# theopaid/Parallel-Image-Convolution-using-MPI-OPENMP-and-CUDA

Hardware: AMD Instinct MI355X
Metric: Mpixels/sec (and wall-time) for 1920x2520 RGB, 40 reps at 1/2/4/8 MI355X (higher is better)
Workload: dtype fp32-exact (packed 16-bit integer, bit-identical to the reference float32)

## Files before the change

### parallel-image-convolution-using-mpi-openmp-and-cuda_amd/csrc/kernels/stencil_swar.hip

```cpp
#include <hip/hip_runtime.h>

#include <algorithm>
#include <cmath>
#include <cstdio>
#include <cstdlib>
#include <atomic>
#include <map>
#include <mutex>
#include <string>
#include <tuple>
#include <type_traits>
#include <vector>

#include "pconv/device.hpp"
#include "swar.hpp"
#include "swar_device.hpp"
#include "tuning.hpp"

namespace pconv {
namespace {

template <int CH, int NP, int M, int NW, int FORM, bool REP>
__device__ __forceinline__ void run_steps(u32 (&D)[M][NP], uint4 (&lds)[2][NW][2][NP / 4][64], int steps, int w,
                                          int lane, bool needs_mask, const u32 (&cm)[NP], int out_top, int out_bot,
                                          const EdgeFix<CH, NP, REP>& ef) {
  if constexpr (REP)
    if (out_top > 0 || out_bot < M) edge_rows<NP, M>(D, out_top, out_bot);
  if constexpr (FORM == 1) {
    int s = 0;
    for (; s + 2 <= steps; s += 2) {
      swar_step<CH, NP, M, NW, 1, REP>(D, lds, 0, w, lane, needs_mask, cm, out_top, out_bot, ef);
      swar_step<CH, NP, M, NW, 2, REP>(D, lds, 1, w, lane, needs_mask, cm, out_top, out_bot, ef);
    }
    if (s < steps) swar_step<CH, NP, M, NW, 0, REP>(D, lds, 0, w, lane, needs_mask, cm, out_top, out_bot, ef);
  } else {
    for (int s = 0; s < steps; ++s)
      swar_step<CH, NP, M, NW, 0, REP>(D, lds, s & 1, w, lane, needs_mask, cm, out_top, out_bot, ef);
  }
}

template <int CH, int NP, int M>
__device__ __forceinline__ void edge_fix(EdgeFix<CH, NP, true>& ef, int baseA, int baseB, bool hasB, int lane,
                                         int row_bytes, int row_base, int g_row0, int height) {
  constexpr int LW = NP;
  edge_masks<CH, NP>(ef, baseA + lane * LW, baseB + lane * LW, hasB, row_bytes);
  const auto holds_edge = [&](int base) {
    return base <= 0 || (base < row_bytes && base + 64 * LW > row_bytes - CH);
  };
  ef.h = holds_edge(baseA) || (hasB && holds_edge(baseB));
  ef.above_own = -g_row0 - row_base == 0;
  ef.below_own = height - 1 - g_row0 - row_base == M - 1;
}
template <int CH, int NP, int M>
__device__ __forceinline__ void edge_fix(EdgeFix<CH, NP, false>&, int, int, bool, int, int, int, int, int) {}

template <int CH, int LW, int M, int NW, int FORM, bool REP = false>
__global__ __launch_bounds__(64 * NW) void k_swar(const uint8_t* __restrict__ src, uint8_t* __restrict__ dst,
                                                  int64_t pitch, int row_bytes, int r0, int r1,
                                                  int steps, int g_row0, int height, int nstrips, int pair_stride,
                                                  int row_tiles, int xcd_swizzle, int tiles_per_image,
                                                  int64_t batch_stride) {
  constexpr int NP = LW;
  constexpr int NQ = NP / 4;
  using CT = typename Chunk<NP>::T;
  __shared__ uint4 lds[2][NW][2][NQ][64];
  const int lane = threadIdx.x & 63;
  const int w = __builtin_amdgcn_readfirstlane(threadIdx.x >> 6);
  const int hl = (steps * CH + LW - 1) / LW;
  const int vbytes = (64 - 2 * hl) * LW;
  int tile = static_cast<int>(blockIdx.x);
  if (xcd_swizzle) {
    const int nwg = static_cast<int>(gridDim.x);
    const int q = nwg >> 3, rem = nwg & 7, xcd = tile & 7, local = tile >> 3;
    tile = xcd * q + min(xcd, rem) + local;
  }
  {
    const int img = tile / tiles_per_image;
    tile -= img * tiles_per_image;
    src += static_cast<int64_t>(img) * batch_stride;
    dst += static_cast<int64_t>(img) * batch_stride;
  }
  const int col = tile / row_tiles, rtile = tile - col * row_tiles;
  const int sA = col, sB = col + pair_stride;
  const bool hasB = sB < nstrips;
  const int baseA = sA * vbytes - hl * LW, baseB = sB * vbytes - hl * LW;
  const int xA = baseA + lane * LW, xB = baseB + lane * LW;
  const int validA = (xA >= 0) ? min(max(row_bytes - xA, 0), LW) : 0;
  const int validB = (hasB && xB >= 0) ? min(max(row_bytes - xB, 0), LW) : 0;
  const bool needs_mask = baseA < 0 || baseA + 64 * LW > row_bytes || !hasB || baseB + 64 * LW > row_bytes;
  u32 cm[NP];
#pragma unroll
  for (int k = 0; k < NP; ++k) cm[k] = (k < validA ? 0xffffu : 0u) | (k < validB ? 0xffff0000u : 0u);

  const int vrows = NW * M - 2 * steps;
  const int tile_r0 = r0 + rtile * vrows;
  const int row_base = tile_r0 - steps + w * M;
  const int lo_ok = max(r0 - steps, -g_row0), hi_ok = min(r1 + steps, height - g_row0);

  u32 D[M][NP];
#pragma unroll
  for (int i = 0; i < M; ++i) {
    const int fr = row_base + i;
    const bool rok = fr >= lo_ok && fr < hi_ok;
    CT a = Chunk<NP>::zero(), b = Chunk<NP>::zero();
    const uint8_t* rowp = src + static_cast<int64_t>(fr) * pitch;
    if (rok && validA > 0) a = *reinterpret_cast<const CT*>(rowp + xA);
    if (rok && validB > 0) b = *reinterpret_cast<const CT*>(rowp + xB);
    unpack<NP>(a, b, D[i]);
  }
  const int out_top = min(max(-g_row0 - row_base, 0), M);
  const int out_bot = min(max(height - g_row0 - row_base, 0), M);

  EdgeFix<CH, NP, REP> ef;
  edge_fix<CH, NP, M>(ef, baseA, baseB, hasB, lane, row_bytes, row_base, g_row0, height);

  run_steps<CH, NP, M, NW, FORM, REP>(D, lds, steps, w, lane, needs_mask, cm, out_top, out_bot, ef);

  const bool lane_in = lane >= hl && lane < 64 - hl;
  const bool stA = lane_in && validA > 0, stB = lane_in && validB > 0;
  const int st_lo = max(tile_r0, r0), st_hi = min(min(tile_r0 + vrows, r1), height - g_row0);
#pragma unroll
  for (int i = 0; i < M; ++i) {
    const int fr = row_base + i;
    if (fr >= st_lo && fr < st_hi) {
      CT a, b;
      pack<NP>(D[i], a, b);
      uint8_t* rowq = dst + static_cast<int64_t>(fr) * pitch;
      if (stA) {
        if (validA == LW)
          *reinterpret_cast<CT*>(rowq + xA) = a;
        else
          store_bytes<NP>(rowq + xA, a, validA);
      }
      if (stB) {
        if (validB == LW)
          *reinterpret_cast<CT*>(rowq + xB) = b;
        else
          store_bytes<NP>(rowq + xB, b, validB);
      }
    }
  }
}

template <int CH, int M, int NW, int FORM, bool REP = false>
__global__ __launch_bounds__(64 * NW) void k_swar_pf(const uint8_t* __restrict__ src, uint8_t* __restrict__ dst,
                                                     int pitch, int row_bytes, int r0, int r1,
                                                     int steps, int g_row0, int height, int nstrips, int pair_stride,
                                                     int row_tiles, int xcd_swizzle, int tiles_per_image,
                                                     int64_t batch_stride) {
  constexpr int LW = 4, NP = 4, NQ = 1;
  constexpr u32 kOut = 0x80000000u;
  __shared__ uint4 lds[2][NW][2][NQ][64];
  const int lane = threadIdx.x & 63;
  const int w = __builtin_amdgcn_readfirstlane(threadIdx.x >> 6);
  const int hl = (steps * CH + LW - 1) / LW;
  const int vbytes = (64 - 2 * hl) * LW;
  const int vrows = NW * M - 2 * steps;
  const int lo_ok = max(r0 - steps, -g_row0), hi_ok = min(r1 + steps, height - g_row0);
  const int st_end = min(r1, height - g_row0);
  int tile = static_cast<int>(blockIdx.x);
  if (xcd_swizzle) {
    const int nwg = static_cast<int>(gridDim.x);
    const int q = nwg >> 3, rem = nwg & 7, xcd = tile & 7, local = tile >> 3;
    tile = xcd * q + min(xcd, rem) + local;
  }
  {
    const int img = tile / tiles_per_image;
    tile -= img * tiles_per_image;
    src += static_cast<int64_t>(img) * batch_stride;
    dst += static_cast<int64_t>(img) * batch_stride;
  }
  const auto srsrc = __builtin_amdgcn_make_buffer_rsrc(
      const_cast<uint8_t*>(src) + static_cast<int64_t>(lo_ok) * pitch, 0, max(hi_ok - lo_ok, 0) * pitch, 0x00020000);
  const auto drsrc = __builtin_amdgcn_make_buffer_rsrc(dst + static_cast<int64_t>(r0) * pitch, 0,
                                                       max(st_end - r0, 0) * pitch, 0x00020000);
  const int col = tile / row_tiles, rtile = tile - col * row_tiles;
  const int sB = col + pair_stride;
  const int baseA = col * vbytes - hl * LW, baseB = sB * vbytes - hl * LW;
  const int pa0 = baseA + lane * LW, pb0 = baseB + lane * LW;
  const int xA = (pa0 >= 0 && pa0 < row_bytes) ? pa0 : -1;
  const int xB = (sB < nstrips && pb0 >= 0 && pb0 < row_bytes) ? pb0 : -1;
  const bool needs_mask = baseA < 0 || baseA + 64 * LW > row_bytes || sB >= nstrips || baseB + 64 * LW > row_bytes;
  const int row_base = r0 + rtile * vrows - steps + w * M;
  u32 D[M][NP];
#pragma unroll
  for (int i = 0; i < M; ++i) {
    const int fr = row_base + i;
    const bool rok = fr >= lo_ok && fr < hi_ok;
    const u32 ro = static_cast<u32>(fr - lo_ok) * static_cast<u32>(pitch);
    const u32 a = __builtin_amdgcn_raw_buffer_load_b32(srsrc, (rok && xA >= 0) ? ro + xA : kOut, 0, 0);
    const u32 b = __builtin_amdgcn_raw_buffer_load_b32(srsrc, (rok && xB >= 0) ? ro + xB : kOut, 0, 0);
    unpack<NP>(a, b, D[i]);
  }
  u32 cm[NP];
#pragma unroll
  for (int k = 0; k < NP; ++k)
    cm[k] = (xA >= 0 && xA + k < row_bytes ? 0xffffu : 0u) | (xB >= 0 && xB + k < row_bytes ? 0xffff0000u : 0u);
  const int out_top = min(max(-g_row0 - row_base, 0), M);
  const int out_bot = min(max(height - g_row0 - row_base, 0), M);
  EdgeFix<CH, NP, REP> ef;
  edge_fix<CH, NP, M>(ef, baseA, baseB, sB < nstrips, lane, row_bytes, row_base, g_row0, height);
  run_steps<CH, NP, M, NW, FORM, REP>(D, lds, steps, w, lane, needs_mask, cm, out_top, out_bot, ef);
  const bool lane_in = lane >= hl && lane < 64 - hl;
  const int tile_r0 = row_base + steps - w * M;
  const int st_lo = max(tile_r0, r0), st_hi = min(tile_r0 + vrows, st_end);
#pragma unroll
  for (int i = 0; i < M; ++i) {
    const int fr = row_base + i;
    const bool rst = fr >= st_lo && fr < st_hi;
    const u32 ro = static_cast<u32>(fr - r0) * static_cast<u32>(pitch);
    u32 a, bb;
    pack<NP>(D[i], a, bb);
    __builtin_amdgcn_raw_buffer_store_b32(a, drsrc, (rst && lane_in && xA >= 0) ? ro + xA : kOut, 0, 0);
    __builtin_amdgcn_raw_buffer_store_b32(bb, drsrc, (rst && lane_in && xB >= 0) ? ro + xB : kOut, 0, 0);
  }
}

struct Tile {
  SwarShape shape;
  bool pf;
};
constexpr Tile kTiles[] = {
    {{8, 8, 8}, false}, {{8, 8, 4}, false}, {{8, 16, 4}, false}, {{8, 4, 8}, false},
    {{4, 8, 8}, true}, {{4, 6, 8}, false}, {{4, 5, 8}, false}, {{4, 4, 8}, false}, {{4, 3, 8}, false},
    {{4, 4, 16}, false},
    {{4, 2, 16}, false}, {{4, 3, 16}, false}, {{8, 2, 16}, false}, {{8, 4, 16}, false},
    {{4, 16, 4}, true}, {{4, 12, 4}, true}, {{4, 16, 8}, true}, {{4, 12, 8}, true},
    {{4, 20, 8}, true},
};
constexpr size_t kNumTiles = sizeof(kTiles) / sizeof(kTiles[0]);

constexpr bool pf_tiles_have_4_byte_lanes() {
  for (const auto& t : kTiles)
    if (t.pf && t.shape.lw != 4) return false;
  return true;
}
static_assert(pf_tiles_have_4_byte_lanes(), "k_swar_pf is written for 4-byte lanes");

size_t tile_index(const SwarShape& s) {
  size_t i = 0;
  while (i < kNumTiles && (kTiles[i].shape.lw != s.lw || kTiles[i].shape.m != s.m || kTiles[i].shape.nw != s.nw)) ++i;
  return i;
}

bool known_shape(const SwarShape& s) { return tile_index(s) < kNumTiles; }

bool known_pf_shape(const SwarShape& s) {
  const size_t i = tile_index(s);
  return i < kNumTiles && kTiles[i].pf;
}

std::atomic<int> g_xcd_swizzle{1};

bool xcd_swizzle_enabled() { return g_xcd_swizzle.load(std::memory_order_relaxed) != 0; }

std::atomic<int> g_alt_mode{-1};

int alt_mode() { return g_alt_mode.load(std::memory_order_relaxed); }

int default_form() { return alt_mode() >= 0 ? alt_mode() : 1; }

std::atomic<int> g_pf_mode{-1};

int pf_mode() { return g_pf_mode.load(std::memory_order_relaxed); }

template <int CH, int LW, int M, int NW>
auto swar_kernel(int form, Border border = Border::Zero) {
  using F = decltype(&k_swar<CH, LW, M, NW, 0>);
  if (border == Border::Replicate)
    return form >= 1 ? static_cast<F>(&k_swar<CH, LW, M, NW, 1, true>)
                     : static_cast<F>(&k_swar<CH, LW, M, NW, 0, true>);
  return form >= 1 ? static_cast<F>(&k_swar<CH, LW, M, NW, 1>) : static_cast<F>(&k_swar<CH, LW, M, NW, 0>);
}

template <int CH, int M, int NW>
auto swar_pf_kernel(int form, Border border = Border::Zero) {
  using F = decltype(&k_swar_pf<CH, M, NW, 0>);
  if (border == Border::Replicate)
    return form >= 1 ? static_cast<F>(&k_swar_pf<CH, M, NW, 1, true>) : static_cast<F>(&k_swar_pf<CH, M, NW, 0, true>);
  return form >= 1 ? static_cast<F>(&k_swar_pf<CH, M, NW, 1>) : static_cast<F>(&k_swar_pf<CH, M, NW, 0>);
}

struct SwarGeom {
  bool ok = false;
  int hl = 0;
  int vbytes = 0;
  int vrows = 0;
  int64_t nstrips = 0, pair_stride = 0, row_tiles = 0;
  int64_t tiles_per_image = 0;
  int64_t tiles = 0;
};

SwarGeom swar_geom(const SwarShape& sh, int ch, int steps, int64_t rows, int64_t row_bytes, int batch = 1) {
  SwarGeom g;
  g.hl = (steps * ch + sh.lw - 1) / sh.lw;
  g.vbytes = (64 - 2 * g.hl) * sh.lw;
  g.vrows = sh.m * sh.nw - 2 * steps;
  g.ok = g.vbytes > 0 && g.vrows > 0 && sh.lw >= ch;
  if (!g.ok) return g;
  g.nstrips = ceil_div<int64_t>(row_bytes, g.vbytes);
  g.pair_stride = (g.nstrips + 1) / 2;
  g.row_tiles = ceil_div<int64_t>(rows, g.vrows);
  g.tiles_per_image = g.pair_stride * g.row_tiles;
  g.tiles = g.tiles_per_image * batch;
  return g;
}

bool pf_launch_ok(const StencilLaunch& a, int steps) {
  const int64_t src_rows = (a.r1 + steps) - (a.r0 - steps), dp = a.pitch;
  return a.row_bytes % 4 == 0 && src_rows * a.pitch < (int64_t(1) << 31) && (a.r1 - a.r0) * dp < (int64_t(1) << 31);
}

template <int CH, size_t I, bool PF>
void launch_tile(const StencilLaunch& a, hipStream_t s, int form) {
  constexpr SwarShape S = kTiles[I].shape;
  const char* who = PF ? "swar prefetch kernel" : "swar temporal kernel";
  const SwarGeom g = swar_geom(S, CH, a.steps, a.r1 - a.r0, a.row_bytes, a.batch);
  PCONV_CHECK(g.ok, std::string(who) + ": steps too large for the tile");
  if constexpr (PF)
    PCONV_CHECK(pf_launch_ok(a, a.steps), std::string(who) + ": needs whole dwords per row and < 2 GiB ranges");
  PCONV_CHECK(g.tiles < (int64_t(1) << 31), std::string(who) + ": too many tiles (batch x tiles per image)");
  const dim3 grid(static_cast<unsigned>(g.tiles)), block(64 * S.nw);
  const int hmax = static_cast<int>(std::min<int64_t>(a.height, int64_t(1) << 30));
  const auto launch = [&](auto kern, auto pitch) {
    kern<<<grid, block, 0, s>>>(a.src, a.dst, pitch, static_cast<int>(a.row_bytes), static_cast<int>(a.r0),
                                static_cast<int>(a.r1), a.steps, static_cast<int>(a.g_row0), hmax,
                                static_cast<int>(g.nstrips), static_cast<int>(g.pair_stride),
                                static_cast<int>(g.row_tiles), xcd_swizzle_enabled() ? 1 : 0,
                                static_cast<int>(g.tiles_per_image), a.batch > 1 ? a.batch_stride : int64_t(0));
  };
  if constexpr (PF)
    launch(swar_pf_kernel<CH, S.m, S.nw>(form, a.border), static_cast<int>(a.pitch));
  else
    launch(swar_kernel<CH, S.lw, S.m, S.nw>(form, a.border), a.pitch);
}

std::mutex g_shape_mu;
bool g_have_shape = false;
SwarShape g_shape;

bool override_shape(SwarShape& out) {
  std::lock_guard<std::mutex> lk(g_shape_mu);
  if (g_have_shape) out = g_shape;
  return g_have_shape;
}

}

void set_swar_shape(int lw, int m, int nw) {
  std::lock_guard<std::mutex> lk(g_shape_mu);
  if (lw == 0) {
    g_have_shape = false;
    return;
  }
  const SwarShape s{lw, m, nw};
  PCONV_CHECK(known_shape(s), "set_swar_shape: shape not instantiated");
  g_shape = s;
  g_have_shape = true;
}

std::vector<SwarShape> swar_shapes() {
  std::vector<SwarShape> out;
  for (const auto& t : kTiles) out.push_back(t.shape);
  return out;
}

std::vector<SwarShape> swar_prefetch_shapes() {
  std::vector<SwarShape> out;
  for (const auto& t : kTiles)
    if (t.pf) out.push_back(t.shape);
  return out;
}

namespace {

struct KernelRes {
  int vgpr = 0;
  int lds = 0;
  bool measured = false;
};

KernelRes query_res(const SwarShape& sh, int ch, int form) {
  hipFuncAttributes at{};
  hipError_t e = hipErrorInvalidValue;
  const bool known = with_channels(static_cast<Channels>(ch), [&](auto chn) {
    return with_index<kNumTiles>(tile_index(sh), [&](auto i) {
      constexpr SwarShape S = kTiles[decltype(i)::value].shape;
      e = hipFuncGetAttributes(
          &at, reinterpret_cast<const void*>(swar_kernel<decltype(chn)::value, S.lw, S.m, S.nw>(form)));
    });
  });
  PCONV_CHECK(known, "swar temporal kernel: unsupported tile shape");
  KernelRes r;
  if (e == hipSuccess && at.numRegs > 0) {
    r.vgpr = at.numRegs;
    r.lds = static_cast<int>(at.sharedSizeBytes);
    r.measured = true;
  } else {
    (void)hipGetLastError();
    r.vgpr = round_up(sh.m * sh.lw + 3 * sh.lw + 40, 8);
    r.lds = sh.nw * sh.lw * 1024;
  }
  return r;
}

KernelRes kernel_res(const SwarShape& sh, int ch, int form) {
  static std::mutex mu;
  static std::map<std::tuple<int, int, int, int, int>, KernelRes> cache;
  std::lock_guard<std::mutex> lk(mu);
  const auto key = std::make_tuple(ch, sh.lw, sh.m, sh.nw, form);
  auto it = cache.find(key);
  if (it != cache.end()) return it->second;
  const KernelRes r = query_res(sh, ch, form);
  if (r.measured) cache.emplace(key, r);
  return r;
}

}

void set_xcd_swizzle(bool on) { g_xcd_swizzle.store(on ? 1 : 0, std::memory_order_relaxed); }
void set_swar_alt(int mode) { g_alt_mode.store(mode < 0 ? -1 : std::min(mode, 1), std::memory_order_relaxed); }
void set_prefetch_mode(int mode) { g_pf_mode.store(mode < 0 ? -1 : mode > 0 ? 1 : 0, std::memory_order_relaxed); }

SwarResources swar_resources(SwarShape s, int ch) {
  const KernelRes r = kernel_res(s, ch, default_form());
  return SwarResources{r.vgpr, r.lds, r.measured};
}

double swar_launch_cycles(SwarShape s, int steps, int ch, int64_t rows, int64_t row_bytes, int batch) {
  constexpr double kCyclesMin = 2.88, kCyclesOneWave = 5.86, kStep = 549.0, kRowLoad = 568.0, kLaunch = 17813.0;
  const int np = s.lw;
  const SwarGeom geom = swar_geom(s, ch, steps, rows, row_bytes, batch);
  if (!geom.ok) return 1e300;
  const double g = static_cast<double>(geom.tiles);
  const KernelRes res = kernel_res(s, ch, default_form());
  const int vgpr_waves = std::max(1, std::min(8, 512 / round_up(std::max(res.vgpr, 1), 8)));
  const int lds_wgs = res.lds > 0 ? (160 * 1024) / res.lds : 8;
  const int L = std::max(1, std::min({lds_wgs, vgpr_waves * 4 / s.nw, 32 / s.nw}));
  const double per_cu = std::ceil(g / 256.0);
  const double rounds = std::ceil(per_cu / L);
  const double k = std::min<double>(per_cu, L) * s.nw / 4.0;
  const double cross = 1.6 * ch;
  const double stage = (s.m + 2) * (2.0 * np + cross) + s.m * 4.0 * np + 24.0;
  const double instr = steps * stage + 40.0 + 3.0 * s.m * np;
  const auto round_cycles = [&](double waves) {
    return instr * std::max(waves * kCyclesMin, kCyclesOneWave) + steps * kStep + kRowLoad * s.m;
  };
  if (batch == 1) return rounds * round_cycles(k) + kLaunch;
  const double full = std::floor(per_cu / L), rest = per_cu - full * L;
  return full * round_cycles(L * s.nw / 4.0) + (rest > 0 ? round_cycles(rest * s.nw / 4.0) : 0.0) + kLaunch;
}

SwarShape pick_swar_shape(int steps, int ch, int64_t rows, int64_t row_bytes, int batch) {
  SwarShape best{0, 0, 0};
  if (override_shape(best) && swar_geom(best, ch, steps, rows, row_bytes).ok) return best;
  double best_cost = 1e300;
  for (const auto& t : kTiles) {
    const double cost = swar_launch_cycles(t.shape, steps, ch, rows, row_bytes, batch);
    if (cost < best_cost) {
      best_cost = cost;
      best = t.shape;
    }
  }
  PCONV_CHECK(best.m > 0, "swar temporal kernel: steps too large for every tile shape");
  return best;
}

namespace {

struct SwarChoice {
  SwarShape shape;
  int form = 1;
  int kern = 0;
};

void launch_choice(const StencilLaunch& a, Channels ch, hipStream_t stream, SwarChoice c) {
  const size_t row = c.kern == 0 || known_pf_shape(c.shape) ? tile_index(c.shape) : kNumTiles;
  const bool known = with_channels(ch, [&](auto chn) {
    return with_index<kNumTiles>(row, [&](auto i) {
      constexpr int CH = decltype(chn)::value;
      constexpr size_t I = decltype(i)::value;
      if (c.kern == 0)
        launch_tile<CH, I, false>(a, stream, c.form);
      else if constexpr (kTiles[I].pf)
        launch_tile<CH, I, true>(a, stream, c.form);
    });
  });
  PCONV_CHECK(known, std::string(c.kern == 0 ? "swar temporal kernel" : "swar prefetch kernel") +
                         ": unsupported tile shape");
}

struct TuneKey {
  int ch, steps;
  int64_t rows, row_bytes;
  int batch;
  bool operator<(const TuneKey& o) const {
    return std::tie(ch, steps, rows, row_bytes, batch) < std::tie(o.ch, o.steps, o.rows, o.row_bytes, o.batch);
  }
};
std::mutex g_tune_mu;
std::map<TuneKey, SwarChoice> g_tuned;
std::atomic<int> g_shape_tuning{1};
std::atomic<int> g_tune_candidates{6};

SwarChoice tuned_choice(const StencilLaunch& a, Channels ch, hipStream_t stream, bool may_measure) {
  const int c = channel_count(ch);
  const int64_t rows = a.r1 - a.r0;
  const int mode = alt_mode();
  const auto runs = [&](const SwarShape& sh) { return swar_geom(sh, c, a.steps, rows, a.row_bytes).tiles > 0; };
  SwarChoice fallback;
  fallback.form = default_form();
  if (pf_mode() == 1 && pf_launch_ok(a, a.steps) && (override_shape(fallback.shape) || !shape_tuning_enabled())) {
    if (!override_shape(fallback.shape) || !known_pf_shape(fallback.shape) || !runs(fallback.shape)) {
      fallback.shape = SwarShape{0, 0, 0};
      for (const auto& t : kTiles)
        if (t.pf && runs(t.shape)) {
          fallback.shape = t.shape;
          break;
        }
    }
    if (fallback.shape.m > 0) {
      fallback.kern = 1;
      return fallback;
    }
    fallback.shape = pick_swar_shape(a.steps, c, rows, a.row_bytes, a.batch);
    return fallback;
  }
  if (override_shape(fallback.shape) || !shape_tuning_enabled()) {
    if (!override_shape(fallback.shape)) fallback.shape = pick_swar_shape(a.steps, c, rows, a.row_bytes, a.batch);
    return fallback;
  }
  const TuneKey key{c, a.steps, rows, a.row_bytes, a.batch};
  {
    std::lock_guard<std::mutex> lk(g_tune_mu);
    auto it = g_tuned.find(key);
    if (it != g_tuned.end()) {
      SwarChoice r = it->second;
      if (mode >= 0) r.form = mode;
      return r;
    }
  }
  fallback.shape = pick_swar_shape(a.steps, c, rows, a.row_bytes, a.batch);
  if (!may_measure || stream_capturing(stream)) return fallback;
  std::vector<std::pair<double, SwarShape>> ranked;
  for (const auto& t : kTiles) {
    const double cost = swar_launch_cycles(t.shape, a.steps, c, rows, a.row_bytes, a.batch);
    if (cost < 1e299) ranked.emplace_back(cost, t.shape);
  }
  PCONV_CHECK(!ranked.empty(), "swar temporal kernel: steps too large for every tile shape");
  std::sort(ranked.begin(), ranked.end(), [](const auto& x, const auto& y) { return x.first < y.first; });
  const size_t keep = static_cast<size_t>(std::max(1, g_tune_candidates.load(std::memory_order_relaxed)));
  if (ranked.size() > keep) ranked.resize(keep);
  std::vector<SwarChoice> cands;
  for (const auto& r : ranked)
    for (int form = 0; form <= 1; ++form)
      if (mode < 0 || mode == form)
        cands.push_back(SwarChoice{r.second, form, 0});
  if (pf_mode() != 0 && pf_launch_ok(a, a.steps)) {
    std::vector<SwarChoice> pfs;
    for (const auto& r : ranked)
      if (known_pf_shape(r.second))
        for (int form = 0; form <= 1; ++form)
          if (mode < 0 || mode == form)
            pfs.push_back(SwarChoice{r.second, form, 1});
    if (pf_mode() == 1 && !pfs.empty()) cands.clear();
    cands.insert(cands.end(), pfs.begin(), pfs.end());
  }
  const SwarChoice best = cands[fastest_candidate(
      cands.size(), stream, [&](size_t i) { launch_choice(a, ch, stream, cands[i]); })];
  std::lock_guard<std::mutex> lk(g_tune_mu);
  g_tuned.emplace(key, best);
  return best;
}

}

void set_tune_candidates(int n) { g_tune_candidates.store(std::max(1, n), std::memory_order_relaxed); }
bool set_shape_tuning(bool on) { return g_shape_tuning.exchange(on ? 1 : 0, std::memory_order_relaxed) != 0; }
bool shape_tuning_enabled() { return g_shape_tuning.load(std::memory_order_relaxed) != 0; }

void clear_swar_tuning() {
  {
    std::lock_guard<std::mutex> lk(g_tune_mu);
    g_tuned.clear();
  }
  clear_float_tuning();
}

std::vector<std::pair<std::vector<int64_t>, SwarShape>> swar_tuned() {
  std::lock_guard<std::mutex> lk(g_tune_mu);
  std::vector<std::pair<std::vector<int64_t>, SwarShape>> out;
  for (const auto& kv : g_tuned)
    out.push_back({{kv.first.ch, kv.first.steps, kv.first.rows, kv.first.row_bytes, kv.second.form,
                    kv.second.kern, kv.first.batch},
                   kv.second.shape});
  return out;
}

namespace {

__global__ __launch_bounds__(256) void k_copy_rows(const uint8_t* __restrict__ src, int64_t sp,
                                                   uint8_t* __restrict__ dst, int64_t dp, int64_t row_bytes,
                                                   int64_t chunks_per_row, int64_t total) {
  const int64_t stride = static_cast<int64_t>(gridDim.x) * blockDim.x;
  for (int64_t i = static_cast<int64_t>(blockIdx.x) * blockDim.x + threadIdx.x; i < total; i += stride) {
    const int64_t y = i / chunks_per_row, x = (i - y * chunks_per_row) * 16;
    const uint8_t* s = src + y * sp + x;
    uint8_t* d = dst + y * dp + x;
    const int n = static_cast<int>(min<int64_t>(16, row_bytes - x));
    const uintptr_t al = reinterpret_cast<uintptr_t>(s) | reinterpret_cast<uintptr_t>(d);
    if (n == 16 && (al & 15) == 0) {
      *reinterpret_cast<uint4*>(d) = *reinterpret_cast<const uint4*>(s);
    } else if (n == 16 && (al & 3) == 0) {
#pragma unroll
      for (int k = 0; k < 4; ++k) reinterpret_cast<u32*>(d)[k] = reinterpret_cast<const u32*>(s)[k];
    } else {
      for (int k = 0; k < n; ++k) d[k] = s[k];
    }
  }
}

__global__ __launch_bounds__(256) void k_fill_zero(uint4* __restrict__ p, int64_t n16) {
  const int64_t stride = static_cast<int64_t>(gridDim.x) * blockDim.x;
  for (int64_t i = static_cast<int64_t>(blockIdx.x) * blockDim.x + threadIdx.x; i < n16; i += stride)
    p[i] = make_uint4(0, 0, 0, 0);
}

unsigned copy_blocks(int64_t work) {
  return static_cast<unsigned>(std::max<int64_t>(1, std::min<int64_t>(ceil_div<int64_t>(work, 256), 2048)));
}

}

void launch_copy_rows(const uint8_t* src, int64_t sp, uint8_t* dst, int64_t dp, int64_t row_bytes, int64_t rows,
                      hipStream_t stream, int max_blocks) {
  PCONV_CHECK(row_bytes >= 0 && rows >= 0 && sp >= row_bytes && dp >= row_bytes, "copy_rows: bad geometry");
  if (row_bytes == 0 || rows == 0) return;
  const int64_t cpr = ceil_div<int64_t>(row_bytes, 16), total = cpr * rows;
  unsigned blocks = copy_blocks(total);
  if (max_blocks > 0) blocks = std::min<unsigned>(blocks, static_cast<unsigned>(max_blocks));
  k_copy_rows<<<dim3(blocks), dim3(256), 0, stream>>>(src, sp, dst, dp, row_bytes, cpr, total);
  PCONV_HIP_CHECK(hipGetLastError());
}

void launch_fill_zero(uint8_t* p, int64_t bytes, hipStream_t stream) {
  PCONV_CHECK(bytes % 16 == 0 && reinterpret_cast<uintptr_t>(p) % 16 == 0, "fill_zero: needs 16-byte granules");
  if (bytes == 0) return;
  k_fill_zero<<<dim3(copy_blocks(bytes / 16)), dim3(256), 0, stream>>>(reinterpret_cast<uint4*>(p), bytes / 16);
  PCONV_HIP_CHECK(hipGetLastError());
}

void preload_kernel_module() {
  hipFuncAttributes at{};
  if (hipFuncGetAttributes(&at, reinterpret_cast<const void*>(&k_fill_zero)) != hipSuccess) (void)hipGetLastError();
}

void prepare_swar(const StencilLaunch& a, Channels ch, hipStream_t stream) { (void)tuned_choice(a, ch, stream, true); }

void launch_swar(const StencilLaunch& a, Channels ch, hipStream_t stream) {
  launch_choice(a, ch, stream, tuned_choice(a, ch, stream, true));
}

}
```

### parallel-image-convolution-using-mpi-openmp-and-cuda_amd/csrc/kernels/swar_device.hpp

```cpp
#pragma once

#include <hip/hip_runtime.h>

#include <cstdint>

namespace pconv {
namespace {

using u32 = uint32_t;

__device__ __forceinline__ u32 perm(u32 hi, u32 lo, u32 sel) { return __builtin_amdgcn_perm(hi, lo, sel); }

__device__ __forceinline__ constexpr u32 pair_sel(int j) {
  return 0x0c000c00u | ((4u + static_cast<u32>(j)) << 16) | static_cast<u32>(j);
}

__device__ __forceinline__ u32 opaque(u32 v) {
  asm volatile("" : "+v"(v));
  return v;
}

__device__ __forceinline__ u32 keep(u32 v) {
  asm("" : "+v"(v));
  return v;
}

template <int DIR>
__device__ __forceinline__ u32 xlane(u32 v) {
  return __builtin_amdgcn_mov_dpp(v, DIR > 0 ? 0x130 : 0x138, 0xf, 0xf, true);
}

template <int CH, int NP>
__device__ __forceinline__ void horiz(const u32 (&X)[NP], u32 (&H)[NP]) {
  static_assert(CH <= NP, "tap distance must not exceed the pairs per lane");
  u32 P[NP];
#pragma unroll
  for (int j = 0; j < NP; ++j)
    P[j] = keep(j + CH < NP ? X[j] + X[j + CH] : xlane<1>(X[j + CH - NP]) + X[j]);
#pragma unroll
  for (int k = 0; k < NP; ++k) H[k] = keep(k >= CH ? P[k - CH] + P[k] : xlane<-1>(P[k - CH + NP]) + P[k]);
}

template <int CH, int NP, bool REP>
struct EdgeFix {};
template <int CH, int NP>
struct EdgeFix<CH, NP, true> {
  u32 eml[CH], emr[NP];
  bool h;
  bool above_own, below_own;
};

template <int CH, int NP>
__device__ __forceinline__ void edge_masks(EdgeFix<CH, NP, true>& e, int pa, int pb, bool hasB, int row_bytes) {
#pragma unroll
  for (int k = 0; k < CH; ++k) e.eml[k] = (pa == 0 ? 0xffffu : 0u) | (hasB && pb == 0 ? 0xffff0000u : 0u);
#pragma unroll
  for (int k = 0; k < NP; ++k) {
    const int ca = pa + k, cb = pb + k;
    e.emr[k] = (ca >= row_bytes - CH && ca < row_bytes && ca >= 0 ? 0xffffu : 0u) |
               (hasB && cb >= row_bytes - CH && cb < row_bytes && cb >= 0 ? 0xffff0000u : 0u);
  }
}

template <int CH, int NP, bool REP>
__device__ __forceinline__ void horiz_b(const u32 (&X)[NP], u32 (&H)[NP], const EdgeFix<CH, NP, REP>& e) {
  horiz<CH, NP>(X, H);
  if constexpr (REP) {
    if (e.h) {
#pragma unroll
      for (int k = 0; k < CH; ++k) H[k] += X[k] & e.eml[k];
#pragma unroll
      for (int k = 0; k < NP; ++k) H[k] += X[k] & e.emr[k];
    }
  }
}

template <int NP>
struct Chunk;
template <>
struct Chunk<8> {
  using T = uint2;
  __device__ static T zero() { return make_uint2(0, 0); }
};
template <>
struct Chunk<4> {
  using T = u32;
  __device__ static T zero() { return 0u; }
};

template <int NP>
__device__ __forceinline__ void unpack(const typename Chunk<NP>::T& a, const typename Chunk<NP>::T& b, u32 (&D)[NP]) {
  if constexpr (NP == 8) {
#pragma unroll
    for (int k = 0; k < 4; ++k) {
      D[k] = perm(b.x, a.x, pair_sel(k));
      D[4 + k] = perm(b.y, a.y, pair_sel(k));
    }
  } else {
#pragma unroll
    for (int k = 0; k < 4; ++k) D[k] = perm(b, a, pair_sel(k));
  }
}

template <int NP>
__device__ __forceinline__ void pack(const u32 (&D)[NP], typename Chunk<NP>::T& a, typename Chunk<NP>::T& b) {
  if constexpr (NP == 8) {
    const u32 t0 = perm(D[1], D[0], 0x06020400u);
    const u32 t1 = perm(D[3], D[2], 0x06020400u);
    const u32 t2 = perm(D[5], D[4], 0x06020400u);
    const u32 t3 = perm(D[7], D[6], 0x06020400u);
    a = make_uint2(perm(t1, t0, 0x05040100u), perm(t3, t2, 0x05040100u));
    b = make_uint2(perm(t1, t0, 0x07060302u), perm(t3, t2, 0x07060302u));
  } else {
    const u32 t0 = perm(D[1], D[0], 0x06020400u);
    const u32 t1 = perm(D[3], D[2], 0x06020400u);
    a = perm(t1, t0, 0x05040100u);
    b = perm(t1, t0, 0x07060302u);
  }
}

template <int NP>
__device__ __forceinline__ void store_bytes(uint8_t* p, const typename Chunk<NP>::T& v, int n) {
  u32 w[2];
  if constexpr (NP == 8) {
    w[0] = v.x;
    w[1] = v.y;
  } else {
    w[0] = v;
    w[1] = 0;
  }
  for (int k = 0; k < n; ++k) p[k] = static_cast<uint8_t>(w[k >> 2] >> (8 * (k & 3)));
}

template <int NP, int M>
__device__ __forceinline__ void edge_rows(u32 (&D)[M][NP], int out_top, int out_bot) {
  out_top = __builtin_amdgcn_readfirstlane(out_top);
  out_bot = __builtin_amdgcn_readfirstlane(out_bot);
  asm volatile("" : "+s"(out_top), "+s"(out_bot));
#pragma unroll
  for (int i = 0; i + 1 < M; ++i) {
    const u32 take = i + 1 == out_top ? 0xffffffffu : 0u;
#pragma unroll
    for (int k = 0; k < NP; ++k) D[i][k] |= D[i + 1][k] & take;
  }
#pragma unroll
  for (int i = M - 1; i >= 1; --i) {
    const u32 take = i == out_bot ? 0xffffffffu : 0u;
#pragma unroll
    for (int k = 0; k < NP; ++k) D[i][k] |= D[i - 1][k] & take;
  }
}

template <int MODE>
__device__ __forceinline__ u32 trunc_sum(u32 S) {
  if constexpr (MODE == 0) return (S >> 4) & 0x00ff00ffu;
  else if constexpr (MODE == 1) return S & 0x0ff00ff0u;
  else return (S >> 8) & 0x00ff00ffu;
}

template <int CH, int NP, int M, int NW, int MODE = 0, bool REP = false>
__device__ __forceinline__ void swar_step(u32 (&D)[M][NP], uint4 (&lds)[2][NW][2][NP / 4][64], int par, int w,
                                             int lane, bool needs_mask, const u32 (&cm)[NP], int out_top,
                                             int out_bot, const EdgeFix<CH, NP, REP>& ef) {
  static_assert(M >= 2, "interior-first step needs two register rows per wave");
  constexpr int NQ = NP / 4;
#pragma unroll
  for (int q = 0; q < NQ; ++q) {
    lds[par][w][0][q][lane] = make_uint4(D[0][4 * q], D[0][4 * q + 1], D[0][4 * q + 2], D[0][4 * q + 3]);
    lds[par][w][1][q][lane] =
        make_uint4(D[M - 1][4 * q], D[M - 1][4 * q + 1], D[M - 1][4 * q + 2], D[M - 1][4 * q + 3]);
  }
  u32 H0[NP], Hc[NP], S01[NP], Sc[NP];
  horiz_b<CH, NP, REP>(D[0], H0, ef);
  horiz_b<CH, NP, REP>(D[1], Hc, ef);
#pragma unroll
  for (int k = 0; k < NP; ++k) {
    S01[k] = keep(H0[k] + Hc[k]);
    Sc[k] = S01[k];
  }
#pragma unroll
  for (int i = 1; i + 1 < M; ++i) {
    u32 Hn[NP];
    horiz_b<CH, NP, REP>(D[i + 1], Hn, ef);
#pragma unroll
    for (int k = 0; k < NP; ++k) {
      const u32 Sn = keep(Hc[k] + Hn[k]);
      D[i][k] = trunc_sum<MODE>(Sc[k] + Sn);
      Sc[k] = Sn;
      Hc[k] = Hn[k];
    }
  }
  __syncthreads();
  {
    int wa = w > 0 ? w - 1 : 0;
    int wb = w < NW - 1 ? w + 1 : w;
    int sa = 1, sb = 0;
    if constexpr (REP) {
      if (ef.above_own) {
        wa = w;
        sa = 0;
      }
      if (ef.below_own) {
        wb = w;
        sb = 1;
      }
    }
    u32 A[NP], B[NP];
#pragma unroll
    for (int q = 0; q < NQ; ++q) {
      const uint4 av = lds[par][wa][sa][q][lane], bv = lds[par][wb][sb][q][lane];
      A[4 * q] = av.x; A[4 * q + 1] = av.y; A[4 * q + 2] = av.z; A[4 * q + 3] = av.w;
      B[4 * q] = bv.x; B[4 * q + 1] = bv.y; B[4 * q + 2] = bv.z; B[4 * q + 3] = bv.w;
    }
    u32 Ha[NP], Hb[NP];
    horiz_b<CH, NP, REP>(A, Ha, ef);
    horiz_b<CH, NP, REP>(B, Hb, ef);
#pragma unroll
    for (int k = 0; k < NP; ++k) {
      D[0][k] = trunc_sum<MODE>(keep(Ha[k] + H0[k]) + S01[k]);
      D[M - 1][k] = trunc_sum<MODE>(Sc[k] + keep(Hc[k] + Hb[k]));
    }
  }
  if (needs_mask) {
#pragma unroll
    for (int i = 0; i < M; ++i)
#pragma unroll
      for (int k = 0; k < NP; ++k) D[i][k] &= cm[k];
  }
  if (out_top > 0 || out_bot < M) {
#pragma unroll
    for (int i = 0; i < M; ++i)
      if (i < out_top || i >= out_bot)
#pragma unroll
        for (int k = 0; k < NP; ++k) D[i][k] = 0;
    if constexpr (REP) edge_rows<NP, M>(D, out_top, out_bot);
  }
}

}
}
```

Baseline: 623,100.

## Publish horizontal sums to LDS and use write-through output stores

Each wave now writes its boundary rows' horizontal partial sums to LDS rather than the raw rows, so neighbours read ready sums and skip the two extra horizontal passes per step. Output stores switch to relaxed agent-scope atomics and buffer stores with a cache-policy bit meant to write through and avoid cache pollution. The LDS publish now happens after the horizontal pass, which may lengthen the path before the barrier. The store policy change could help or hurt depending on cache behaviour.

```diff
diff --git a/parallel-image-convolution-using-mpi-openmp-and-cuda_amd/csrc/kernels/stencil_swar.hip b/parallel-image-convolution-using-mpi-openmp-and-cuda_amd/csrc/kernels/stencil_swar.hip
--- a/parallel-image-convolution-using-mpi-openmp-and-cuda_amd/csrc/kernels/stencil_swar.hip
+++ b/parallel-image-convolution-using-mpi-openmp-and-cuda_amd/csrc/kernels/stencil_swar.hip
@@ -128,13 +128,13 @@
       uint8_t* rowq = dst + static_cast<int64_t>(fr) * pitch;
       if (stA) {
         if (validA == LW)
-          *reinterpret_cast<CT*>(rowq + xA) = a;
+          store_through(rowq + xA, a);
         else
           store_bytes<NP>(rowq + xA, a, validA);
       }
       if (stB) {
         if (validB == LW)
-          *reinterpret_cast<CT*>(rowq + xB) = b;
+          store_through(rowq + xB, b);
         else
           store_bytes<NP>(rowq + xB, b, validB);
       }
@@ -211,8 +211,8 @@
     const u32 ro = static_cast<u32>(fr - r0) * static_cast<u32>(pitch);
     u32 a, bb;
     pack<NP>(D[i], a, bb);
-    __builtin_amdgcn_raw_buffer_store_b32(a, drsrc, (rst && lane_in && xA >= 0) ? ro + xA : kOut, 0, 0);
-    __builtin_amdgcn_raw_buffer_store_b32(bb, drsrc, (rst && lane_in && xB >= 0) ? ro + xB : kOut, 0, 0);
+    __builtin_amdgcn_raw_buffer_store_b32(a, drsrc, (rst && lane_in && xA >= 0) ? ro + xA : kOut, 0, kWriteThrough);
+    __builtin_amdgcn_raw_buffer_store_b32(bb, drsrc, (rst && lane_in && xB >= 0) ? ro + xB : kOut, 0, kWriteThrough);
   }
 }
 
diff --git a/parallel-image-convolution-using-mpi-openmp-and-cuda_amd/csrc/kernels/swar_device.hpp b/parallel-image-convolution-using-mpi-openmp-and-cuda_amd/csrc/kernels/swar_device.hpp
--- a/parallel-image-convolution-using-mpi-openmp-and-cuda_amd/csrc/kernels/swar_device.hpp
+++ b/parallel-image-convolution-using-mpi-openmp-and-cuda_amd/csrc/kernels/swar_device.hpp
@@ -119,6 +119,15 @@
   }
 }
 
+constexpr int kWriteThrough = 16;
+__device__ __forceinline__ void store_through(uint8_t* p, u32 v) {
+  __hip_atomic_store(reinterpret_cast<u32*>(p), v, __ATOMIC_RELAXED, __HIP_MEMORY_SCOPE_AGENT);
+}
+__device__ __forceinline__ void store_through(uint8_t* p, uint2 v) {
+  __hip_atomic_store(reinterpret_cast<unsigned long long*>(p), (static_cast<unsigned long long>(v.y) << 32) | v.x,
+                     __ATOMIC_RELAXED, __HIP_MEMORY_SCOPE_AGENT);
+}
+
 template <int NP>
 __device__ __forceinline__ void store_bytes(uint8_t* p, const typename Chunk<NP>::T& v, int n) {
   u32 w[2];
@@ -164,14 +173,14 @@
                                              int out_bot, const EdgeFix<CH, NP, REP>& ef) {
   static_assert(M >= 2, "interior-first step needs two register rows per wave");
   constexpr int NQ = NP / 4;
-#pragma unroll
-  for (int q = 0; q < NQ; ++q) {
-    lds[par][w][0][q][lane] = make_uint4(D[0][4 * q], D[0][4 * q + 1], D[0][4 * q + 2], D[0][4 * q + 3]);
-    lds[par][w][1][q][lane] =
-        make_uint4(D[M - 1][4 * q], D[M - 1][4 * q + 1], D[M - 1][4 * q + 2], D[M - 1][4 * q + 3]);
-  }
+  const auto publish = [&](int slot, const u32(&H)[NP]) {
+#pragma unroll
+    for (int q = 0; q < NQ; ++q)
+      lds[par][w][slot][q][lane] = make_uint4(H[4 * q], H[4 * q + 1], H[4 * q + 2], H[4 * q + 3]);
+  };
   u32 H0[NP], Hc[NP], S01[NP], Sc[NP];
   horiz_b<CH, NP, REP>(D[0], H0, ef);
+  publish(0, H0);
   horiz_b<CH, NP, REP>(D[1], Hc, ef);
 #pragma unroll
   for (int k = 0; k < NP; ++k) {
@@ -190,6 +199,7 @@
       Hc[k] = Hn[k];
     }
   }
+  publish(1, Hc);
   __syncthreads();
   {
     int wa = w > 0 ? w - 1 : 0;
@@ -205,16 +215,13 @@
         sb = 1;
       }
     }
-    u32 A[NP], B[NP];
+    u32 Ha[NP], Hb[NP];
 #pragma unroll
     for (int q = 0; q < NQ; ++q) {
       const uint4 av = lds[par][wa][sa][q][lane], bv = lds[par][wb][sb][q][lane];
-      A[4 * q] = av.x; A[4 * q + 1] = av.y; A[4 * q + 2] = av.z; A[4 * q + 3] = av.w;
-      B[4 * q] = bv.x; B[4 * q + 1] = bv.y; B[4 * q + 2] = bv.z; B[4 * q + 3] = bv.w;
-    }
-    u32 Ha[NP], Hb[NP];
-    horiz_b<CH, NP, REP>(A, Ha, ef);
-    horiz_b<CH, NP, REP>(B, Hb, ef);
+      Ha[4 * q] = av.x; Ha[4 * q + 1] = av.y; Ha[4 * q + 2] = av.z; Ha[4 * q + 3] = av.w;
+      Hb[4 * q] = bv.x; Hb[4 * q + 1] = bv.y; Hb[4 * q + 2] = bv.z; Hb[4 * q + 3] = bv.w;
+    }
 #pragma unroll
     for (int k = 0; k < NP; ++k) {
       D[0][k] = trunc_sum<MODE>(keep(Ha[k] + H0[k]) + S01[k]);
```

Result: no change. 625,900 (median of 3 runs) (+0.4%).
